# toposware/schnorr-sig

Measured on NVIDIA B200. Metric: schnorr_verifications_per_sec, higher is better.
Workload: dtype u64 (Goldilocks Fp / Fp6 on 32-bit IMAD, exact)

## Files before the change

schnorr-sig_b200/csrc/schnorr_b200.cu:

```cuda
#include <cuda_runtime.h>

#include <cstdio>
#include <cstdlib>
#include <cstring>
#include <string>
#include <vector>

#include "../../include/cheetah_params.h"
#include "../../include/schnorr_b200.h"
#include "verify.cuh"
#include "keyset.cuh"
#include "dist.cuh"
#include "debug_ops.cuh"
#include "derive.cuh"

using namespace sb;

static constexpr size_t GTAB_U64 = (size_t)GTAB_WINDOWS * GTAB_ENTRIES * 12;
static constexpr size_t REG_BATCH_MIN_PER_KEY = 64;

enum scratch_slot { SL_A = 0, SL_B, SL_C, SL_D, SL_E, SL_F, SL_G, SL_H, SL_I, SL_J, SL_K, SL_L, SL_M, SL_N, SL_O, SL_COUNT };

struct schnorr_b200_ctx {
    int device = 0;
    cudaStream_t stream = nullptr;
    cudaStream_t own_stream = nullptr;
    uint64_t* gtab = nullptr;
    void* scratch[SL_COUNT] = {};
    size_t scratch_cap[SL_COUNT] = {};
    uint64_t launches = 0;
    int sm_count = 148;
    cudaEvent_t ev_k0 = nullptr, ev_k1 = nullptr;
    size_t verify_wave = 148 * 256;
    cudaStream_t copy_stream = nullptr;
    cudaStream_t aux_stream = nullptr;
    cudaEvent_t ev_aux = nullptr;
    bool exact_only = false;
    int msm_c_override = 0;
    uint32_t msm_t_override = 0;
    int last_msm_c = 0, last_msm_K = 0;
    uint32_t last_msm_T = 0;
    uint64_t last_batch_points = 0;
    size_t reg_batch_min_per_key = REG_BATCH_MIN_PER_KEY;
    size_t dist_max = 10240;
    size_t one_max = 512;
    size_t batch_dist_max = (size_t)1 << 18;
    size_t batch_small_max = 256;
    int exact_counters_used = 0;
    static constexpr int MAX_CHUNKS = 16;
    cudaEvent_t ev_chunk[MAX_CHUNKS] = {};
    std::string err;
    std::vector<schnorr_b200_ctx*> shards;
};

#define CUDA_TRY(ctx, expr)                                                                      \
    do {                                                                                         \
        cudaError_t e_ = (expr);                                                                 \
        if (e_ != cudaSuccess) {                                                                 \
            (ctx)->err = std::string(#expr) + ": " + cudaGetErrorString(e_);                     \
            return SCHNORR_B200_ECUDA;                                                           \
        }                                                                                        \
    } while (0)

static int ensure_scratch(schnorr_b200_ctx* ctx, int slot, size_t bytes, void** out) {
    if (bytes == 0) bytes = 16;
    if (ctx->scratch_cap[slot] < bytes) {
        if (ctx->scratch[slot]) {
            CUDA_TRY(ctx, cudaStreamSynchronize(ctx->stream));
            CUDA_TRY(ctx, cudaFree(ctx->scratch[slot]));
            ctx->scratch[slot] = nullptr;
            ctx->scratch_cap[slot] = 0;
        }
        size_t cap = bytes + bytes / 8;
        CUDA_TRY(ctx, cudaMalloc(&ctx->scratch[slot], cap));
        ctx->scratch_cap[slot] = cap;
    }
    *out = ctx->scratch[slot];
    return 0;
}

static constexpr uint8_t FL_PK_INF = 1;
static constexpr uint8_t FL_X_BAD = 2;
static constexpr uint8_t FL_MALFORMED = 4;
static constexpr int SOA_PLANES = 11;

struct soa_batch {
    ulonglong2* planes;
    uint8_t* flags;
    uint8_t* sig_flag;
    size_t n;
};

__device__ __forceinline__ ulonglong2 load_plane(const ulonglong2* p) {
    return __ldcs(p);
}
__device__ __forceinline__ fp6 load_fp6_planes(const ulonglong2* planes, int first_plane, size_t n, size_t i) {
    ulonglong2 a = load_plane(&planes[(size_t)(first_plane + 0) * n + i]);
    ulonglong2 b = load_plane(&planes[(size_t)(first_plane + 1) * n + i]);
    ulonglong2 c = load_plane(&planes[(size_t)(first_plane + 2) * n + i]);
    return fp6{{a.x, a.y, b.x, b.y, c.x, c.y}};
}
__device__ __forceinline__ scalar load_scalar_planes(const ulonglong2* planes, int first_plane, size_t n, size_t i) {
    ulonglong2 a = load_plane(&planes[(size_t)(first_plane + 0) * n + i]);
    ulonglong2 b = load_plane(&planes[(size_t)(first_plane + 1) * n + i]);
    return sc_from_u64x4(a.x, a.y, b.x, b.y);
}
__device__ __forceinline__ uint64_t load_u64_le(const uint8_t* p) {
    uint64_t v = 0;
#pragma unroll
    for (int k = 0; k < 8; k++) v |= (uint64_t)p[k] << (8 * k);
    return v;
}

struct hash_vote {
    bool sync, any;
};
__device__ __forceinline__ hash_vote block_hash_vote(int np, uint64_t& off, uint64_t& len) {
    __shared__ int s_np_min, s_np_max, s_first;
    __shared__ uint64_t s_off, s_len;
    if (threadIdx.x == 0) {
        s_np_min = 1 << 30;
        s_np_max = -1;
        s_first = 1 << 30;
    }
    __syncthreads();
    if (np >= 0) {
        atomicMin(&s_np_min, np);
        atomicMax(&s_np_max, np);
        atomicMin(&s_first, (int)threadIdx.x);
    }
    __syncthreads();
    if ((int)threadIdx.x == s_first) {
        s_off = off;
        s_len = len;
    }
    __syncthreads();
    hash_vote v;
    v.any = s_np_max >= 0;
    v.sync = v.any && s_np_min >= s_np_max;
    if (np < 0 && v.any) {
        off = s_off;
        len = s_len;
    }
    return v;
}

static constexpr int INGEST_THREADS = 128;
__global__ void __launch_bounds__(INGEST_THREADS) k_ingest(size_t n, const uint8_t* __restrict__ sigs81,
                                                           const uint8_t* __restrict__ pk96,
                                                           const uint8_t* __restrict__ pk_inf, soa_batch out) {
    __shared__ __align__(16) uint8_t s_sig[INGEST_THREADS * 81];
    size_t base = (size_t)blockIdx.x * INGEST_THREADS;
    size_t cnt = n - base < (size_t)INGEST_THREADS ? n - base : (size_t)INGEST_THREADS;
    size_t bytes = cnt * 81;
    const uint8_t* src = sigs81 + base * 81;
    if ((reinterpret_cast<uintptr_t>(src) & 15) == 0) {
        size_t nv = bytes / 16;
        for (size_t k = threadIdx.x; k < nv; k += INGEST_THREADS)
            reinterpret_cast<uint4*>(s_sig)[k] = reinterpret_cast<const uint4*>(src)[k];
        for (size_t k = nv * 16 + threadIdx.x; k < bytes; k += INGEST_THREADS) s_sig[k] = src[k];
    } else {
        for (size_t k = threadIdx.x; k < bytes; k += INGEST_THREADS) s_sig[k] = src[k];
    }
    __syncthreads();
    size_t i = base + threadIdx.x;
    if (i >= n) return;
    const uint8_t* rec = s_sig + threadIdx.x * 81;
    uint64_t x[6], e[4];
#pragma unroll
    for (int k = 0; k < 6; k++) x[k] = load_u64_le(rec + 8 * k);
#pragma unroll
    for (int k = 0; k < 4; k++) e[k] = load_u64_le(rec + 49 + 8 * k);
    const uint64_t* pk = reinterpret_cast<const uint64_t*>(pk96 + i * 96);
    uint64_t p[12];
#pragma unroll
    for (int k = 0; k < 12; k++) p[k] = pk[k];
    uint8_t fl = 0;
    bool inf = pk_inf != nullptr && pk_inf[i] != 0;
    if (inf) fl |= FL_PK_INF;
    bool x_ok = true, pk_ok = true;
#pragma unroll
    for (int k = 0; k < 6; k++) x_ok &= x[k] < FP_P;
#pragma unroll
    for (int k = 0; k < 12; k++) pk_ok &= p[k] < FP_P;
    if (!x_ok) fl |= FL_X_BAD;
    if ((!pk_ok && !inf) || sc_geq_q(sc_from_u64x4(e[0], e[1], e[2], e[3]))) fl |= FL_MALFORMED;
    size_t N = out.n;
    ulonglong2* pl = out.planes;
    pl[0 * N + i] = make_ulonglong2(x[0], x[1]);
    pl[1 * N + i] = make_ulonglong2(x[2], x[3]);
    pl[2 * N + i] = make_ulonglong2(x[4], x[5]);
    pl[3 * N + i] = make_ulonglong2(e[0], e[1]);
    pl[4 * N + i] = make_ulonglong2(e[2], e[3]);
#pragma unroll
    for (int k = 0; k < 6; k++) pl[(size_t)(5 + k) * N + i] = make_ulonglong2(p[2 * k], p[2 * k + 1]);
    out.flags[i] = fl;
    out.sig_flag[i] = rec[48];
}

#ifndef VERIFY_THREADS_N
#define VERIFY_THREADS_N 128
#endif
static constexpr int VERIFY_THREADS = VERIFY_THREADS_N;
#ifndef VERIFY_MIN_BLOCKS
#define VERIFY_MIN_BLOCKS 2
#endif
__global__ void __launch_bounds__(VERIFY_THREADS, VERIFY_MIN_BLOCKS) k_verify(soa_batch in, const uint8_t* __restrict__ msgs,
                                                           const uint64_t* __restrict__ msg_off,
                                                           const uint64_t* __restrict__ gtab,
                                                           uint8_t* __restrict__ verdicts,
                                                           const uint32_t* __restrict__ work_list,
                                                           const uint32_t* __restrict__ work_count) {
    struct d_slot {
        jac_pt p;
        uint64_t pad;
    };
    __shared__ d_slot s_d[VERIFY_THREADS];
    size_t i = (size_t)blockIdx.x * blockDim.x + threadIdx.x;
    if (work_list) {
        if (i >= *work_count) return;
        i = work_list[i];
    }
    if (i >= in.n) return;
    uint8_t fl = in.flags[i];
    if (fl & FL_MALFORMED) {
        verdicts[i] = VERDICT_MALFORMED;
        return;
    }
    fp6 sx = load_fp6_planes(in.planes, 0, in.n, i);
    scalar e = load_scalar_planes(in.planes, 3, in.n, i);
    fp6 px = load_fp6_planes(in.planes, 5, in.n, i);
    fp6 py = load_fp6_planes(in.planes, 8, in.n, i);
    bool pk_inf = fl & FL_PK_INF;
    bool x_ok = !(fl & FL_X_BAD);
    uint64_t off = msg_off[i];
    scalar h = sc_zero();
    if (x_ok) h = challenge_scalar(sx, px, py, pk_inf, msgs + off, msg_off[i + 1] - off);
    verdicts[i] = verify_points(sx, x_ok, e, px, py, pk_inf, h, gtab, &s_d[threadIdx.x].p);
}

#ifndef VERIFY_FAST_MIN_BLOCKS
#define VERIFY_FAST_MIN_BLOCKS 2
#endif
static constexpr size_t VERIFY_FAST_SMEM = (size_t)(1 + FAST_BH_SHARED) * VERIFY_THREADS * sizeof(jf_pt);
__global__ void __launch_bounds__(VERIFY_THREADS, VERIFY_FAST_MIN_BLOCKS) k_verify_fast(soa_batch in, const uint8_t* __restrict__ msgs,
                                                           const uint64_t* __restrict__ msg_off,
                                                           const uint64_t* __restrict__ gtab,
                                                           uint8_t* __restrict__ verdicts,
                                                           uint32_t* __restrict__ work_list,
                                                           uint32_t* __restrict__ work_count) {
    extern __shared__ __align__(16) unsigned char s_fast[];
    jf_pt* s_d = reinterpret_cast<jf_pt*>(s_fast);
    jf_pt* s_bh = s_d + VERIFY_THREADS;
    size_t i = (size_t)blockIdx.x * blockDim.x + threadIdx.x;
    bool live = i < in.n;
    uint8_t fl = live ? in.flags[i] : FL_MALFORMED;
    bool work = live && !(fl & (FL_MALFORMED | FL_PK_INF));
    uint64_t off = work ? msg_off[i] : 0, len = work ? msg_off[i + 1] - off : 0;
    hash_vote hv = block_hash_vote(work ? hash_message_permutations(len) : -1, off, len);
    fp6 sx = fp6_zero(), px, py;
    scalar e = sc_zero();
    if (work) {
        sx = load_fp6_planes(in.planes, 0, in.n, i);
        e = load_scalar_planes(in.planes, 3, in.n, i);
        px = load_fp6_planes(in.planes, 5, in.n, i);
        py = load_fp6_planes(in.planes, 8, in.n, i);
    } else {
        const uint64_t* g = gtab + (size_t)1 * GTAB_ENTRY_U64;
#pragma unroll
        for (int k = 0; k < 6; k++) {
            px.c[k] = g[k];
            py.c[k] = g[6 + k];
        }
    }
    bool x_ok = !(fl & FL_X_BAD);
    scalar h = sc_zero();
    if (hv.any) {
        h = challenge_scalar(sx, px, py, false, msgs + off, len, hv.sync);
        if (!x_ok || !work) h = sc_zero();
    }
    uint8_t v = verify_points_fast(sx, x_ok, e, px, py, false, h, gtab, s_d + threadIdx.x, s_bh + threadIdx.x, VERIFY_THREADS);
    if (!live) return;
    if (fl & FL_MALFORMED) v = VERDICT_MALFORMED;
    else if (fl & FL_PK_INF) v = VERDICT_NEEDS_EXACT;
    verdicts[i] = v;
    if (v == VERDICT_NEEDS_EXACT) work_list[atomicAdd(work_count, 1u)] = (uint32_t)i;
}

static constexpr int DIST_THREADS = 128;
static constexpr int DIST_SIGS_PER_BLOCK = (DIST_THREADS / 32) * 5;
__global__ void __launch_bounds__(DIST_THREADS) k_verify_dist(soa_batch in, const uint8_t* __restrict__ msgs,
                                                              const uint64_t* __restrict__ msg_off,
                                                              const uint64_t* __restrict__ gtab,
                                                              uint8_t* __restrict__ verdicts,
                                                              uint32_t* __restrict__ work_list,
                                                              uint32_t* __restrict__ work_count) {
    __shared__ uint32_t s_mds2[24];
    if (threadIdx.x < 24) s_mds2[threadIdx.x] = c_mds_row[threadIdx.x % 12];
    __syncthreads();
    int lane = threadIdx.x & 31, warp = threadIdx.x >> 5;
    int g = lane / 6, k = lane % 6;
    if (g >= 5) return;
    size_t i = ((size_t)blockIdx.x * (DIST_THREADS / 32) + warp) * 5 + g;
    if (i >= in.n) return;
    int gbase = 6 * g;
    unsigned mask = 0x3fu << gbase;
    uint8_t fl = in.flags[i];
    if (fl & FL_MALFORMED) {
        if (k == 0) verdicts[i] = VERDICT_MALFORMED;
        return;
    }
    uint8_t v;
    if (fl & FL_PK_INF) {
        v = VERDICT_NEEDS_EXACT;
    } else {
        bool x_ok = !(fl & FL_X_BAD);
        const uint64_t* pl = reinterpret_cast<const uint64_t*>(in.planes);
        size_t n = in.n;
        fp_t sx = pl[((size_t)(0 + (k >> 1)) * n + i) * 2 + (k & 1)];
        fp_t px = pl[((size_t)(5 + (k >> 1)) * n + i) * 2 + (k & 1)];
        fp_t py = pl[((size_t)(8 + (k >> 1)) * n + i) * 2 + (k & 1)];
        scalar e = load_scalar_planes(in.planes, 3, n, i);
        uint64_t off = msg_off[i];
        scalar h = sc_zero();
        if (x_ok) h = dchallenge_scalar(mask, sx, px, py, msgs + off, msg_off[i + 1] - off, k, gbase, s_mds2);
        dpt r;
        int fr = dverify_core(mask, px, py, h, e, gtab, &r, k, gbase);
        bool eq = dall(mask, gbase, r.X == fp_mul(sx, fp_sqr_nc(r.w)));
        v = fr == FAST_EXCEPTIONAL ? VERDICT_NEEDS_EXACT
            : (fr == FAST_NOT_TORSION_FREE ? VERDICT_INVALID_PUBLIC_KEY
               : (!x_ok ? VERDICT_MALFORMED : (eq ? VERDICT_OK : VERDICT_INVALID_SIGNATURE)));
    }
    if (k == 0) {
        verdicts[i] = v;
        if (v == VERDICT_NEEDS_EXACT) work_list[atomicAdd(work_count, 1u)] = (uint32_t)i;
    }
}


static constexpr int HASH_THREADS = 128;
__global__ void __launch_bounds__(HASH_THREADS) k_hash(size_t n, const uint8_t* __restrict__ rx48,
                                                       const uint8_t* __restrict__ pk96,
                                                       const uint8_t* __restrict__ msgs,
                                                       const uint64_t* __restrict__ msg_off,
                                                       uint8_t* __restrict__ digests) {
    size_t i = (size_t)blockIdx.x * blockDim.x + threadIdx.x;
    bool live = i < n;
    uint64_t off = live ? msg_off[i] : 0, len = live ? msg_off[i + 1] - off : 0;
    hash_vote hv = block_hash_vote(live ? hash_message_permutations(len) : -1, off, len);
    size_t src = live ? i : (size_t)blockIdx.x * blockDim.x;
    const uint64_t* r = reinterpret_cast<const uint64_t*>(rx48 + src * 48);
    const uint64_t* p = reinterpret_cast<const uint64_t*>(pk96 + src * 96);
    fp6 rx, px;
#pragma unroll
    for (int k = 0; k < 6; k++) {
        rx.c[k] = r[k];
        px.c[k] = p[k];
    }
    fp_t py0 = p[6];
    fp_t d[4];
    hash_message(rx, px, py0, msgs + off, len, d, hv.sync);
    if (!live) return;
    ulonglong2* o = reinterpret_cast<ulonglong2*>(digests + i * 32);
    o[0] = make_ulonglong2(d[0], d[1]);
    o[1] = make_ulonglong2(d[2], d[3]);
}

__global__ void __launch_bounds__(DIST_THREADS) k_hash_dist(size_t n, const uint8_t* __restrict__ rx48,
                                                            const uint8_t* __restrict__ pk96,
                                                            const uint8_t* __restrict__ msgs,
                                                            const uint64_t* __restrict__ msg_off,
                                                            uint8_t* __restrict__ digests) {
    __shared__ uint32_t s_mds2[24];
    if (threadIdx.x < 24) s_mds2[threadIdx.x] = c_mds_row[threadIdx.x % 12];
    __syncthreads();
    int lane = threadIdx.x & 31, warp = threadIdx.x >> 5;
    int g = lane / 6, k = lane % 6;
    if (g >= 5) return;
    size_t i = ((size_t)blockIdx.x * (DIST_THREADS / 32) + warp) * 5 + g;
    if (i >= n) return;
    int gbase = 6 * g;
    unsigned mask = 0x3fu << gbase;
    const uint64_t* r = reinterpret_cast<const uint64_t*>(rx48 + i * 48);
    const uint64_t* p = reinterpret_cast<const uint64_t*>(pk96 + i * 96);
    uint64_t off = msg_off[i];
    fp_t d[4];
    dhash_message(mask, r[k], p[k], p[6 + k], msgs + off, msg_off[i + 1] - off, k, gbase, s_mds2, d);
    if (k < 4) reinterpret_cast<uint64_t*>(digests + i * 32)[k] = d[k];
}

static constexpr int SIGN_THREADS = 128;
__device__ __forceinline__ void store_point96(uint8_t* dst, const fp6& x, const fp6& y) {
    uint64_t* o = reinterpret_cast<uint64_t*>(dst);
#pragma unroll
    for (int k = 0; k < 6; k++) {
        o[k] = x.c[k];
        o[6 + k] = y.c[k];
    }
}
__global__ void __launch_bounds__(SIGN_THREADS) k_keygen(size_t n, const uint8_t* __restrict__ sk32,
                                                         const uint64_t* __restrict__ gtab, uint8_t* __restrict__ pk96,
                                                         uint8_t* __restrict__ pk_inf) {
    size_t i = (size_t)blockIdx.x * blockDim.x + threadIdx.x;
    if (i >= n) return;
    scalar k = sc_from_u256(sc_load_le(sk32 + 32 * i));
    jac_pt P = fixed_base_mul(k, gtab);
    fp6 x, y;
    bool inf;
    jac_to_affine(P, x, y, inf);
    store_point96(pk96 + 96 * i, x, y);
    if (pk_inf) pk_inf[i] = inf ? 1 : 0;
}
__global__ void __launch_bounds__(SIGN_THREADS) k_sign(size_t n, const uint8_t* __restrict__ sk32,
                                                       const uint8_t* __restrict__ pk96,
                                                       const uint8_t* __restrict__ pk_inf,
                                                       const uint8_t* __restrict__ msgs,
                                                       const uint64_t* __restrict__ msg_off,
                                                       const uint8_t* __restrict__ nonce32,
                                                       const uint64_t* __restrict__ gtab, uint8_t* __restrict__ sigs81) {
    size_t i = (size_t)blockIdx.x * blockDim.x + threadIdx.x;
    if (i >= n) return;
    scalar sk = sc_from_u256(sc_load_le(sk32 + 32 * i));
    scalar r = sc_from_u256(sc_load_le(nonce32 + 32 * i));
    const uint64_t* p = reinterpret_cast<const uint64_t*>(pk96 + i * 96);
    fp6 px, py;
#pragma unroll
    for (int k = 0; k < 6; k++) {
        px.c[k] = p[k];
        py.c[k] = p[6 + k];
    }
    bool inf = pk_inf != nullptr && pk_inf[i] != 0;
    jac_pt R = fixed_base_mul(r, gtab);
    fp6 x, y;
    bool r_inf;
    jac_to_affine(R, x, y, r_inf);
    uint64_t off = msg_off[i];
    scalar h = challenge_scalar(x, px, py, inf, msgs + off, msg_off[i + 1] - off);
    scalar e = sc_sub(r, sc_mul(sk, h));
    uint8_t* o = sigs81 + 81 * i;
#pragma unroll
    for (int k = 0; k < 6; k++)
#pragma unroll
        for (int b = 0; b < 8; b++) o[8 * k + b] = (uint8_t)(x.c[k] >> (8 * b));
    o[48] = compress_flags(y, r_inf);
#pragma unroll
    for (int k = 0; k < 8; k++)
#pragma unroll
        for (int b = 0; b < 4; b++) o[49 + 4 * k + b] = (uint8_t)(e.l[k] >> (8 * b));
}

__global__ void __launch_bounds__(128) k_decompress(size_t n, const uint8_t* __restrict__ in49, uint8_t* __restrict__ pk96,
                                                    uint8_t* __restrict__ pk_inf, uint8_t* __restrict__ ok) {
    size_t i = (size_t)blockIdx.x * blockDim.x + threadIdx.x;
    if (i >= n) return;
    const uint8_t* rec = in49 + 49 * i;
    fp6 x;
#pragma unroll
    for (int k = 0; k < 6; k++) x.c[k] = load_u64_le(rec + 8 * k);
    fp6 ox, oy;
    bool inf;
    bool good = decompress_point(x, rec[48], ox, oy, inf);
    store_point96(pk96 + 96 * i, ox, oy);
    pk_inf[i] = inf ? 1 : 0;
    ok[i] = good ? 1 : 0;
}
__global__ void __launch_bounds__(128) k_compress(size_t n, const uint8_t* __restrict__ pk96,
                                                  const uint8_t* __restrict__ pk_inf, uint8_t* __restrict__ out49) {
    size_t i = (size_t)blockIdx.x * blockDim.x + threadIdx.x;
    if (i >= n) return;
    const uint64_t* p = reinterpret_cast<const uint64_t*>(pk96 + i * 96);
    bool inf = pk_inf != nullptr && pk_inf[i] != 0;
    fp6 y;
#pragma unroll
    for (int k = 0; k < 6; k++) y.c[k] = p[6 + k];
    uint8_t* o = out49 + 49 * i;
#pragma unroll
    for (int k = 0; k < 6; k++) {
        uint64_t v = inf ? 0 : p[k];
#pragma unroll
        for (int b = 0; b < 8; b++) o[8 * k + b] = (uint8_t)(v >> (8 * b));
    }
    o[48] = compress_flags(y, inf);
}

__global__ void __launch_bounds__(128) k_split_keyed(size_t n, const uint8_t* __restrict__ keyed130, uint8_t* __restrict__ pk96,
                                                     uint8_t* __restrict__ pk_inf, uint8_t* __restrict__ ok,
                                                     uint8_t* __restrict__ sigs81) {
    size_t i = (size_t)blockIdx.x * blockDim.x + threadIdx.x;
    if (i >= n) return;
    const uint8_t* rec = keyed130 + 130 * i;
    fp6 x;
#pragma unroll
    for (int k = 0; k < 6; k++) x.c[k] = load_u64_le(rec + 8 * k);
    fp6 ox, oy;
    bool inf;
    bool good = decompress_point(x, rec[48], ox, oy, inf);
    store_point96(pk96 + 96 * i, ox, oy);
    pk_inf[i] = inf ? 1 : 0;
    ok[i] = good ? 1 : 0;
    for (int k = 0; k < 81; k++) sigs81[81 * i + k] = rec[49 + k];
}
__global__ void k_mask_verdicts(size_t n, const uint8_t* __restrict__ ok, uint8_t* __restrict__ verdicts) {
    size_t i = (size_t)blockIdx.x * blockDim.x + threadIdx.x;
    if (i < n && !ok[i]) verdicts[i] = VERDICT_MALFORMED;
}

__global__ void __launch_bounds__(128) k_derive_master(size_t n, const uint8_t* __restrict__ seeds32, uint8_t* __restrict__ xsk64,
                                                       uint8_t* __restrict__ ok) {
    size_t i = (size_t)blockIdx.x * blockDim.x + threadIdx.x;
    if (i >= n) return;
    ok[i] = derive_master(seeds32 + 32 * i, xsk64 + 64 * i) ? 1 : 0;
}
__global__ void __launch_bounds__(128) k_derive_private(size_t n, const uint8_t* __restrict__ parent_xsk64,
                                                        const uint8_t* __restrict__ parent49, const uint32_t* __restrict__ indices,
                                                        uint8_t* __restrict__ children64, uint8_t* __restrict__ ok) {
    size_t i = (size_t)blockIdx.x * blockDim.x + threadIdx.x;
    if (i >= n) return;
    ok[i] = derive_private_child(parent_xsk64, parent49, indices[i], children64 + 64 * i) ? 1 : 0;
}
__global__ void k_parent_public(const uint8_t* __restrict__ parent_xsk64, const uint64_t* __restrict__ gtab, uint8_t* __restrict__ out49) {
    if (blockIdx.x != 0 || threadIdx.x != 0) return;
    scalar k = sc_from_u256(sc_load_le(parent_xsk64));
    jac_pt P = fixed_base_mul(k, gtab);
    fp6 x, y;
    bool inf;
    jac_to_affine(P, x, y, inf);
    for (int c = 0; c < 6; c++)
        for (int b = 0; b < 8; b++) out49[8 * c + b] = (uint8_t)((inf ? 0 : x.c[c]) >> (8 * b));
    out49[48] = compress_flags(y, inf);
}
__global__ void __launch_bounds__(SIGN_THREADS) k_derive_public(size_t n, const uint8_t* __restrict__ parent_xpk81,
                                                                const uint8_t* __restrict__ parent96,
                                                                const uint8_t* __restrict__ parent_inf,
                                                                const uint32_t* __restrict__ indices,
                                                                const uint64_t* __restrict__ gtab, uint8_t* __restrict__ children81,
                                                                uint8_t* __restrict__ ok) {
    size_t i = (size_t)blockIdx.x * blockDim.x + threadIdx.x;
    if (i >= n) return;
    uint32_t index = indices[i];
    uint8_t* o = children81 + 81 * i;
    scalar t = derive_public_tweak(parent_xpk81, parent_xpk81 + 49, index, o + 49);
    const uint64_t* p = reinterpret_cast<const uint64_t*>(parent96);
    fp6 px, py;
#pragma unroll
    for (int k = 0; k < 6; k++) {
        px.c[k] = p[k];
        py.c[k] = p[6 + k];
    }
    jac_pt acc = fixed_base_mul(t, gtab);
    bool tweak_inf = jac_is_identity(acc);
    acc = jac_madd(acc, px, py, parent_inf[0] != 0);
    fp6 x, y;
    bool inf;
    jac_to_affine(acc, x, y, inf);
#pragma unroll
    for (int k = 0; k < 6; k++)
#pragma unroll
        for (int b = 0; b < 8; b++) o[8 * k + b] = (uint8_t)((inf ? 0 : x.c[k]) >> (8 * b));
    o[48] = compress_flags(y, inf);
    ok[i] = (!tweak_inf && (index >> 31) == 0) ? 1 : 0;
}

__global__ void __launch_bounds__(128) k_tab_bases(size_t n_pts, const uint64_t* __restrict__ pts12, const uint8_t* __restrict__ skip,
                                                   int w, int windows, jac_pt* __restrict__ bases) {
    size_t p = (size_t)blockIdx.x * blockDim.x + threadIdx.x;
    if (p >= n_pts || (skip && skip[p])) return;
    tab_bases(pts12 + 12 * p, w, windows, bases + p * windows);
}
__global__ void __launch_bounds__(128) k_tab_fill(size_t n_pts, const uint8_t* __restrict__ skip, int w, int windows,
                                                  const jac_pt* __restrict__ bases, uint64_t* __restrict__ tab) {
    size_t t = (size_t)blockIdx.x * blockDim.x + threadIdx.x;
    size_t entries = ((size_t)1 << (w - 1)) + 1, per_pt = (size_t)windows * entries;
    if (t >= n_pts * per_pt) return;
    size_t p = t / per_pt;
    if (skip && skip[p]) return;
    tab_entry(bases[t / entries], w, (int)(t % entries), tab + t * 12);
}

__global__ void __launch_bounds__(128) k_keyset_register(size_t n_keys, const uint64_t* __restrict__ pk12,
                                                         const uint8_t* __restrict__ pk_inf, uint8_t* __restrict__ status,
                                                         uint8_t* __restrict__ skip) {
    size_t k = (size_t)blockIdx.x * blockDim.x + threadIdx.x;
    if (k >= n_keys) return;
    bool inf = pk_inf[k] != 0;
    jac_pt d;
    uint8_t st = keyset_key_status(pk12 + 12 * k, inf, &d);
    status[k] = st;
    skip[k] = st != KEY_OK || inf;
}
__global__ void __launch_bounds__(128) k_keyset_gather(size_t n, const uint32_t* __restrict__ key_idx, size_t n_keys,
                                                       const uint64_t* __restrict__ ks_pk12, const uint8_t* __restrict__ ks_inf,
                                                       uint64_t* __restrict__ pk12, uint8_t* __restrict__ pk_inf) {
    size_t i = (size_t)blockIdx.x * blockDim.x + threadIdx.x;
    if (i >= n) return;
    uint32_t k = key_idx[i];
    bool in = k < n_keys;
#pragma unroll
    for (int c = 0; c < 12; c++) pk12[12 * i + c] = in ? ks_pk12[12 * (size_t)k + c] : ~0ULL;
    pk_inf[i] = in ? ks_inf[k] : 0;
}
__global__ void __launch_bounds__(128) k_keyset_encode(size_t n_keys, const uint64_t* __restrict__ pk12,
                                                       const uint8_t* __restrict__ pk_inf, keyset_entry* __restrict__ entries,
                                                       uint8_t* __restrict__ findable) {
    size_t k = (size_t)blockIdx.x * blockDim.x + threadIdx.x;
    if (k >= n_keys) return;
    keyset_entry e;
    uint8_t flag;
    findable[k] = keyset_encode(pk12 + 12 * k, pk_inf[k] != 0, e.x, flag) ? 1 : 0;
    e.flag = flag;
    e.index = (uint32_t)k;
    e.pad = 0;
    entries[k] = e;
}
__global__ void __launch_bounds__(128) k_keyset_lookup(size_t n, const uint8_t* __restrict__ keys49,
                                                       const keyset_entry* __restrict__ lut, uint32_t n_lut,
                                                       uint32_t* __restrict__ key_idx) {
    size_t i = (size_t)blockIdx.x * blockDim.x + threadIdx.x;
    if (i >= n) return;
    const uint8_t* rec = keys49 + 49 * i;
    uint64_t x[6];
#pragma unroll
    for (int k = 0; k < 6; k++) x[k] = load_u64_le(rec + 8 * k);
    key_idx[i] = keyset_lookup(lut, n_lut, x, rec[48]);
}
__global__ void __launch_bounds__(128) k_keyed_split_lookup(size_t n, const uint8_t* __restrict__ keyed130,
                                                            const keyset_entry* __restrict__ lut, uint32_t n_lut,
                                                            const uint64_t* __restrict__ ks_pk12,
                                                            const uint8_t* __restrict__ ks_inf, uint8_t* __restrict__ pk96,
                                                            uint8_t* __restrict__ pk_inf, uint8_t* __restrict__ ok,
                                                            uint8_t* __restrict__ sigs81, uint32_t* __restrict__ key_idx,
                                                            uint32_t* __restrict__ miss_count) {
    size_t i = (size_t)blockIdx.x * blockDim.x + threadIdx.x;
    bool miss = false;
    if (i < n) {
        const uint8_t* rec = keyed130 + 130 * i;
        fp6 x;
#pragma unroll
        for (int k = 0; k < 6; k++) x.c[k] = load_u64_le(rec + 8 * k);
        uint32_t k = keyset_lookup(lut, n_lut, x.c, rec[48]);
        miss = k == KEYSET_MISS;
        if (!miss) {
            uint64_t* o = reinterpret_cast<uint64_t*>(pk96 + 96 * i);
#pragma unroll
            for (int c = 0; c < 12; c++) o[c] = ks_pk12[12 * (size_t)k + c];
            pk_inf[i] = ks_inf[k];
            ok[i] = 1;
        } else {
            fp6 ox, oy;
            bool inf;
            bool good = decompress_point(x, rec[48], ox, oy, inf);
            store_point96(pk96 + 96 * i, ox, oy);
            pk_inf[i] = inf ? 1 : 0;
            ok[i] = good ? 1 : 0;
        }
        key_idx[i] = k;
        for (int c = 0; c < 81; c++) sigs81[81 * i + c] = rec[49 + c];
    }
    unsigned m = __ballot_sync(0xffffffffu, miss);
    if ((threadIdx.x & 31) == 0 && m) atomicAdd(miss_count, (unsigned)__popc(m));
}

template <bool LOOKUP>
__global__ void __launch_bounds__(VERIFY_THREADS) k_verify_reg(soa_batch in, const uint32_t* __restrict__ key_idx,
                                                               const uint8_t* __restrict__ key_status,
                                                               const uint64_t* __restrict__ ktab,
                                                               const uint8_t* __restrict__ msgs,
                                                               const uint64_t* __restrict__ msg_off,
                                                               const uint64_t* __restrict__ gtab,
                                                               uint8_t* __restrict__ verdicts,
                                                               uint32_t* __restrict__ work_list,
                                                               uint32_t* __restrict__ work_count) {
    size_t i = (size_t)blockIdx.x * blockDim.x + threadIdx.x;
    bool live = i < in.n;
    uint8_t fl = live ? in.flags[i] : FL_MALFORMED;
    bool keyed = !(fl & (FL_MALFORMED | FL_PK_INF));
    uint32_t k = keyed ? key_idx[i] : 0;
    bool miss = LOOKUP && k == KEYSET_MISS;
    if (miss) {
        keyed = false;
        k = 0;
    }
    uint8_t st = keyed ? key_status[k] : KEY_OK;
    bool work = keyed && st == KEY_OK;
    uint64_t off = work ? msg_off[i] : 0, len = work ? msg_off[i + 1] - off : 0;
    hash_vote hv = block_hash_vote(work ? hash_message_permutations(len) : -1, off, len);
    fp6 sx = fp6_zero(), px, py;
    scalar e = sc_zero();
    if (work) {
        sx = load_fp6_planes(in.planes, 0, in.n, i);
        e = load_scalar_planes(in.planes, 3, in.n, i);
        px = load_fp6_planes(in.planes, 5, in.n, i);
        py = load_fp6_planes(in.planes, 8, in.n, i);
    } else {
        const uint64_t* g = gtab + (size_t)1 * GTAB_ENTRY_U64;
#pragma unroll
        for (int c = 0; c < 6; c++) {
            px.c[c] = g[c];
            py.c[c] = g[6 + c];
        }
    }
    bool x_ok = !(fl & FL_X_BAD);
    scalar h = sc_zero();
    if (hv.any) {
        h = challenge_scalar(sx, px, py, false, msgs + off, len, hv.sync);
        if (!x_ok || !work) h = sc_zero();
    }
    jf_pt r;
    int fr = verify_core_reg(h, e, ktab + (size_t)k * KT_KEY_U64, gtab, &r);
    if (!live) return;
    uint8_t v;
    if (fl & FL_MALFORMED) v = VERDICT_MALFORMED;
    else if (fl & FL_PK_INF) v = VERDICT_NEEDS_EXACT;
    else if (miss) v = VERDICT_NEEDS_EXACT;
    else v = reg_verdict(st, x_ok, fr, r, sx);
    verdicts[i] = v;
    if (v == VERDICT_NEEDS_EXACT) work_list[atomicAdd(work_count, 1u)] = (uint32_t)i;
}

__global__ void __launch_bounds__(128) k_debug_field(size_t n, const uint64_t* __restrict__ a6, const uint64_t* __restrict__ b6,
                                                     uint64_t* __restrict__ out48) {
    size_t i = (size_t)blockIdx.x * blockDim.x + threadIdx.x;
    if (i >= n) return;
    fp6 a, b;
#pragma unroll
    for (int k = 0; k < 6; k++) {
        a.c[k] = a6[i * 6 + k];
        b.c[k] = b6[i * 6 + k];
    }
    fp6 m = fp6_mul(a, b), q = fp6_sqr(a), ad = fp6_add(a, b), su = fp6_sub(a, b), iv = fp6_inv(a);
    uint64_t* o = out48 + i * 48;
#pragma unroll
    for (int k = 0; k < 6; k++) {
        o[k] = m.c[k];
        o[6 + k] = q.c[k];
        o[12 + k] = ad.c[k];
        o[18 + k] = su.c[k];
        o[24 + k] = fp_mul(a.c[k], b.c[k]);
        o[30 + k] = fp_sqr(a.c[k]);
        o[36 + k] = iv.c[k];
        o[42 + k] = rescue_inv_sbox(a.c[k]);
    }
}

__global__ void __launch_bounds__(128) k_debug_lazy(size_t n, const uint64_t* __restrict__ a6, const uint64_t* __restrict__ b6,
                                                    uint64_t* __restrict__ out48) {
    size_t i = (size_t)blockIdx.x * blockDim.x + threadIdx.x;
    if (i >= n) return;
    fp6 a, b, r[8];
#pragma unroll
    for (int k = 0; k < 6; k++) {
        a.c[k] = a6[i * 6 + k];
        b.c[k] = b6[i * 6 + k];
    }
    debug_lazy_ops(a, b, r);
    for (int j = 0; j < 8; j++)
        for (int k = 0; k < 6; k++) out48[i * 48 + 6 * j + k] = r[j].c[k];
}

__global__ void __launch_bounds__(256) k_imad_peak(int iters, uint64_t* sink) {
    uint32_t a = threadIdx.x * 2654435761u + 12345u, b = blockIdx.x * 40503u + 977u;
    uint64_t acc[8];
#pragma unroll
    for (int k = 0; k < 8; k++) acc[k] = k;
    for (int it = 0; it < iters; it++) {
#pragma unroll
        for (int k = 0; k < 8; k++) {
            asm volatile("mad.wide.u32 %0, %1, %2, %0;" : "+l"(acc[k]) : "r"(a + k), "r"(b));
        }
        b += 3;
    }
    uint64_t s = 0;
#pragma unroll
    for (int k = 0; k < 8; k++) s ^= acc[k];
    if (s == 0x123456789abcdefULL) sink[0] = s;
}

static inline unsigned grid_for(size_t n, int threads) { return (unsigned)((n + threads - 1) / threads); }

static int build_tables(schnorr_b200_ctx* ctx, size_t n_pts, const uint64_t* pts12, const uint8_t* skip, int w, int windows,
                        jac_pt* bases, uint64_t* tab) {
    size_t threads = n_pts * (size_t)windows * (((size_t)1 << (w - 1)) + 1);
    k_tab_bases<<<grid_for(n_pts, 128), 128, 0, ctx->stream>>>(n_pts, pts12, skip, w, windows, bases);
    k_tab_fill<<<grid_for(threads, 128), 128, 0, ctx->stream>>>(n_pts, skip, w, windows, bases, tab);
    ctx->launches += 2;
    CUDA_TRY(ctx, cudaGetLastError());
    return 0;
}

static int alloc_soa(schnorr_b200_ctx* ctx, size_t n, soa_batch* b) {
    void *p, *f, *sf;
    if (int rc = ensure_scratch(ctx, SL_A, sizeof(ulonglong2) * SOA_PLANES * n, &p)) return rc;
    if (int rc = ensure_scratch(ctx, SL_B, n, &f)) return rc;
    if (int rc = ensure_scratch(ctx, SL_C, n, &sf)) return rc;
    b->planes = (ulonglong2*)p;
    b->flags = (uint8_t*)f;
    b->sig_flag = (uint8_t*)sf;
    b->n = n;
    return 0;
}

static bool msg_off_valid(size_t n, const uint64_t* msg_off) {
    if (msg_off[0] != 0) return false;
    for (size_t i = 0; i < n; i++)
        if (msg_off[i + 1] < msg_off[i]) return false;
    return true;
}
#define CHECK_MSG_OFF(ctx, n, msg_off)                                                            \
    do {                                                                                          \
        if (!msg_off_valid((n), (msg_off))) {                                                     \
            (ctx)->err = "message offsets must start at 0 and be non-decreasing";                 \
            return SCHNORR_B200_EARG;                                                             \
        }                                                                                         \
    } while (0)

static int stage_in(schnorr_b200_ctx* ctx, int slot, const void* host, size_t bytes, void** dev) {
    if (int rc = ensure_scratch(ctx, slot, bytes, dev)) return rc;
    if (host && bytes) CUDA_TRY(ctx, cudaMemcpyAsync(*dev, host, bytes, cudaMemcpyHostToDevice, ctx->stream));
    return 0;
}

#define MULTI_DISPATCH(ctx, call)                                  \
    do {                                                           \
        if ((ctx) && !(ctx)->shards.empty()) return call;          \
    } while (0)
#define NOT_ON_MULTI(ctx)                                                                                          \
    do {                                                                                                           \
        if ((ctx) && !(ctx)->shards.empty()) {                                                                     \
            (ctx)->err = "device-pointer entry points need a single-device context (buffers live on one device)"; \
            return SCHNORR_B200_EARG;                                                                              \
        }                                                                                                          \
    } while (0)

static int verify_many_host(schnorr_b200_ctx* ctx, size_t n, const uint8_t* sigs81, const uint8_t* pk96, const uint8_t* pk_inf,
                            const uint8_t* msgs, const uint64_t* msg_off, uint8_t* verdicts, bool validate_offsets);
#include "batch.cuh"
#include "multi.cuh"
#include "one.cuh"


static int launch_verify(schnorr_b200_ctx* ctx, const soa_batch& soa, const uint8_t* msgs, const uint64_t* msg_off,
                         uint8_t* verdicts, size_t list_base, int counter, size_t list_total, cudaStream_t st) {
    unsigned grid = grid_for(soa.n, VERIFY_THREADS);
    if (counter == 0) ctx->exact_counters_used = 0;
    if (ctx->exact_only) {
        k_verify<<<grid, VERIFY_THREADS, 0, st>>>(soa, msgs, msg_off, ctx->gtab, verdicts, nullptr, nullptr);
        ctx->launches += 1;
        return 0;
    }
    void* wl;
    if (int rc = ensure_scratch(ctx, SL_M, 4 * (list_total + schnorr_b200_ctx::MAX_CHUNKS), &wl)) return rc;
    uint32_t* counters = (uint32_t*)wl;
    uint32_t* list = counters + schnorr_b200_ctx::MAX_CHUNKS + list_base;
    CUDA_TRY(ctx, cudaMemsetAsync(counters + counter, 0, 4, st));
    if (counter + 1 > ctx->exact_counters_used) ctx->exact_counters_used = counter + 1;
    if (soa.n <= ctx->one_max)
        if (soa.n <= (size_t)2 * ctx->sm_count)
            k_verify_one<2><<<(unsigned)soa.n, ONE_THREADS, 0, st>>>(soa, msgs, msg_off, ctx->gtab, verdicts, list, counters + counter);
        else
            k_verify_one<4><<<(unsigned)soa.n, ONE_THREADS, 0, st>>>(soa, msgs, msg_off, ctx->gtab, verdicts, list, counters + counter);
    else if (soa.n <= ctx->dist_max)
        k_verify_dist<<<grid_for(soa.n, DIST_SIGS_PER_BLOCK), DIST_THREADS, 0, st>>>(soa, msgs, msg_off, ctx->gtab, verdicts, list,
                                                                                   counters + counter);
    else
        k_verify_fast<<<grid, VERIFY_THREADS, VERIFY_FAST_SMEM, st>>>(soa, msgs, msg_off, ctx->gtab, verdicts, list, counters + counter);
    k_verify<<<grid, VERIFY_THREADS, 0, st>>>(soa, msgs, msg_off, ctx->gtab, verdicts, list, counters + counter);
    ctx->launches += 2;
    return 0;
}

extern "C" {

int schnorr_b200_params_pinned(void) { return CHEETAH_PARAMS_PINNED; }
const char* schnorr_b200_params_provenance(void) { return CHEETAH_PARAMS_PROVENANCE; }

int schnorr_b200_create(int device, schnorr_b200_ctx** out) {
    if (!out) return SCHNORR_B200_EARG;
    *out = nullptr;
#if !CHEETAH_PARAMS_PINNED
    {
        static bool warned = false;
        if (!warned) {
            warned = true;
            fprintf(stderr, "schnorr_b200: curve / hash parameters are NOT pinned to the upstream cheetah / hash crates (%s). "
                            "Keys and signatures interoperate with the real schnorr-sig crate only after "
                            "rust/dump_params has been run and include/cheetah_params.h regenerated.\n",
                    CHEETAH_PARAMS_PROVENANCE);
        }
    }
#endif
    int count = 0;
    if (cudaGetDeviceCount(&count) != cudaSuccess || count <= 0 || device < 0 || device >= count) {
        (void)cudaGetLastError();
        return SCHNORR_B200_ENODEV;
    }
    schnorr_b200_ctx* ctx = new schnorr_b200_ctx();
    ctx->device = device;
    auto fail = [&](int rc) {
        fprintf(stderr, "schnorr_b200_create: %s\n", ctx->err.c_str());
        schnorr_b200_destroy(ctx);
        return rc;
    };
#define CREATE_TRY(expr)                                                          \
    do {                                                                          \
        cudaError_t e_ = (expr);                                                  \
        if (e_ != cudaSuccess) {                                                  \
            ctx->err = std::string(#expr) + ": " + cudaGetErrorString(e_);        \
            return fail(SCHNORR_B200_ECUDA);                                      \
        }                                                                         \
    } while (0)
    CREATE_TRY(cudaSetDevice(device));
    cudaDeviceProp prop;
    CREATE_TRY(cudaGetDeviceProperties(&prop, device));
    ctx->sm_count = prop.multiProcessorCount;
    CREATE_TRY(cudaStreamCreateWithFlags(&ctx->own_stream, cudaStreamNonBlocking));
    ctx->stream = ctx->own_stream;
    {
        int per_sm = 0;
        CREATE_TRY(cudaFuncSetAttribute(k_verify_fast, cudaFuncAttributeMaxDynamicSharedMemorySize, (int)VERIFY_FAST_SMEM));
        CREATE_TRY(cudaFuncSetAttribute(k_verify_fast, cudaFuncAttributePreferredSharedMemoryCarveout, cudaSharedmemCarveoutMaxShared));
        CREATE_TRY(cudaOccupancyMaxActiveBlocksPerMultiprocessor(&per_sm, k_verify_fast, VERIFY_THREADS, VERIFY_FAST_SMEM));
        if (per_sm < 1) per_sm = 1;
        ctx->verify_wave = (size_t)ctx->sm_count * per_sm * VERIFY_THREADS;
    }
    CREATE_TRY(cudaStreamCreateWithFlags(&ctx->copy_stream, cudaStreamNonBlocking));
    CREATE_TRY(cudaStreamCreateWithFlags(&ctx->aux_stream, cudaStreamNonBlocking));
    CREATE_TRY(cudaEventCreateWithFlags(&ctx->ev_aux, cudaEventDisableTiming));
    for (int c = 0; c < schnorr_b200_ctx::MAX_CHUNKS; c++) CREATE_TRY(cudaEventCreateWithFlags(&ctx->ev_chunk[c], cudaEventDisableTiming));
    CREATE_TRY(cudaEventCreate(&ctx->ev_k0));
    CREATE_TRY(cudaEventCreate(&ctx->ev_k1));
    CREATE_TRY(cudaMemcpyToSymbol(c_ark, RESCUE_ARK, sizeof(uint64_t) * 2 * RESCUE_ROUNDS * 12));
    CREATE_TRY(cudaMemcpyToSymbol(c_q_wnaf5, CHEETAH_Q_WNAF5, sizeof(CHEETAH_Q_WNAF5)));
    CREATE_TRY(cudaMemcpyToSymbol(c_q_wnaf4, CHEETAH_Q_WNAF4, 256));
    CREATE_TRY(cudaMalloc(&ctx->gtab, GTAB_U64 * sizeof(uint64_t)));
    jac_pt* bases = nullptr;
    CREATE_TRY(cudaMalloc(&bases, sizeof(jac_pt) * GTAB_WINDOWS + 96));
    uint64_t* g12 = reinterpret_cast<uint64_t*>(bases + GTAB_WINDOWS);
    CREATE_TRY(cudaMemcpyAsync(g12, CHEETAH_GX, 48, cudaMemcpyHostToDevice, ctx->stream));
    CREATE_TRY(cudaMemcpyAsync(g12 + 6, CHEETAH_GY, 48, cudaMemcpyHostToDevice, ctx->stream));
    if (build_tables(ctx, 1, g12, nullptr, GTAB_W, GTAB_WINDOWS, bases, ctx->gtab)) {
        cudaFree(bases);
        return fail(SCHNORR_B200_ECUDA);
    }
    CREATE_TRY(cudaStreamSynchronize(ctx->stream));
    cudaFree(bases);
#undef CREATE_TRY
    *out = ctx;
    return SCHNORR_B200_OK;
}

int schnorr_b200_create_multi(const int* devices, int n_devices, schnorr_b200_ctx** out) {
    if (!out) return SCHNORR_B200_EARG;
    *out = nullptr;
    if (!devices || n_devices <= 0 || n_devices > 64) return SCHNORR_B200_EARG;
    if (n_devices == 1) return schnorr_b200_create(devices[0], out);
    schnorr_b200_ctx* ctx = new schnorr_b200_ctx();
    ctx->device = devices[0];
    for (int k = 0; k < n_devices; k++) {
        schnorr_b200_ctx* sh = nullptr;
        int rc = schnorr_b200_create(devices[k], &sh);
        if (rc != SCHNORR_B200_OK) {
            schnorr_b200_destroy(ctx);
            return rc;
        }
        ctx->shards.push_back(sh);
    }
    ctx->sm_count = ctx->shards[0]->sm_count;
    ctx->verify_wave = ctx->shards[0]->verify_wave;
    *out = ctx;
    return SCHNORR_B200_OK;
}
int schnorr_b200_device_count(const schnorr_b200_ctx* ctx) { return !ctx ? 0 : (ctx->shards.empty() ? 1 : (int)ctx->shards.size()); }

void schnorr_b200_destroy(schnorr_b200_ctx* ctx) {
    if (!ctx) return;
    if (!ctx->shards.empty()) {
        for (schnorr_b200_ctx* sh : ctx->shards) schnorr_b200_destroy(sh);
        delete ctx;
        return;
    }
    cudaSetDevice(ctx->device);
    if (ctx->own_stream) cudaStreamSynchronize(ctx->own_stream);
    for (int s = 0; s < SL_COUNT; s++)
        if (ctx->scratch[s]) cudaFree(ctx->scratch[s]);
    if (ctx->gtab) cudaFree(ctx->gtab);
    for (int c = 0; c < schnorr_b200_ctx::MAX_CHUNKS; c++)
        if (ctx->ev_chunk[c]) cudaEventDestroy(ctx->ev_chunk[c]);
    if (ctx->copy_stream) cudaStreamDestroy(ctx->copy_stream);
    if (ctx->aux_stream) cudaStreamDestroy(ctx->aux_stream);
    if (ctx->ev_aux) cudaEventDestroy(ctx->ev_aux);
    if (ctx->ev_k0) cudaEventDestroy(ctx->ev_k0);
    if (ctx->ev_k1) cudaEventDestroy(ctx->ev_k1);
    if (ctx->own_stream) cudaStreamDestroy(ctx->own_stream);
    delete ctx;
}

const char* schnorr_b200_last_error(const schnorr_b200_ctx* ctx) { return ctx ? ctx->err.c_str() : "null context"; }

int schnorr_b200_set_stream(schnorr_b200_ctx* ctx, void* stream) {
    if (!ctx) return SCHNORR_B200_EARG;
    NOT_ON_MULTI(ctx);
    ctx->stream = stream ? (cudaStream_t)stream : ctx->own_stream;
    return SCHNORR_B200_OK;
}
int schnorr_b200_synchronize(schnorr_b200_ctx* ctx) {
    if (!ctx) return SCHNORR_B200_EARG;
    for (schnorr_b200_ctx* sh : ctx->shards)
        if (int rc = schnorr_b200_synchronize(sh)) return rc;
    if (!ctx->shards.empty()) return SCHNORR_B200_OK;
    CUDA_TRY(ctx, cudaStreamSynchronize(ctx->stream));
    return SCHNORR_B200_OK;
}
uint64_t schnorr_b200_launch_count(const schnorr_b200_ctx* ctx) {
    if (!ctx) return 0;
    uint64_t total = ctx->launches;
    for (const schnorr_b200_ctx* sh : ctx->shards) total += sh->launches;
    return total;
}
int schnorr_b200_last_kernel_ms(schnorr_b200_ctx* ctx, float* ms) {
    if (!ctx || !ms) return SCHNORR_B200_EARG;
    if (!ctx->shards.empty()) {
        *ms = 0;
        for (schnorr_b200_ctx* sh : ctx->shards) {
            float m = 0;
            if (int rc = schnorr_b200_last_kernel_ms(sh, &m)) return rc;
            if (m > *ms) *ms = m;
        }
        return SCHNORR_B200_OK;
    }
    CUDA_TRY(ctx, cudaEventSynchronize(ctx->ev_k1));
    CUDA_TRY(ctx, cudaEventElapsedTime(ms, ctx->ev_k0, ctx->ev_k1));
    return SCHNORR_B200_OK;
}

int schnorr_b200_set_exact_only(schnorr_b200_ctx* ctx, int exact_only) {
    if (!ctx) return SCHNORR_B200_EARG;
    for (schnorr_b200_ctx* sh : ctx->shards) sh->exact_only = exact_only != 0;
    ctx->exact_only = exact_only != 0;
    return SCHNORR_B200_OK;
}
int schnorr_b200_set_dist_threshold(schnorr_b200_ctx* ctx, size_t max_signatures) {
    if (!ctx) return SCHNORR_B200_EARG;
    for (schnorr_b200_ctx* sh : ctx->shards) sh->dist_max = max_signatures;
    ctx->dist_max = max_signatures;
    return SCHNORR_B200_OK;
}
int schnorr_b200_set_one_threshold(schnorr_b200_ctx* ctx, size_t max_signatures) {
    if (!ctx) return SCHNORR_B200_EARG;
    for (schnorr_b200_ctx* sh : ctx->shards) sh->one_max = max_signatures;
    ctx->one_max = max_signatures;
    return SCHNORR_B200_OK;
}
int schnorr_b200_set_batch_small_threshold(schnorr_b200_ctx* ctx, size_t max_signatures) {
    if (!ctx) return SCHNORR_B200_EARG;
    for (schnorr_b200_ctx* sh : ctx->shards) sh->batch_small_max = max_signatures;
    ctx->batch_small_max = max_signatures;
    return SCHNORR_B200_OK;
}
int schnorr_b200_set_batch_dist_threshold(schnorr_b200_ctx* ctx, size_t max_signatures) {
    if (!ctx) return SCHNORR_B200_EARG;
    ctx->batch_dist_max = max_signatures;
    for (schnorr_b200_ctx* sh : ctx->shards) sh->batch_dist_max = max_signatures;
    return SCHNORR_B200_OK;
}
int schnorr_b200_set_msm_geometry(schnorr_b200_ctx* ctx, int window_bits, unsigned segment_len) {
    if (!ctx || (window_bits != 0 && (window_bits < 4 || window_bits > 16)) || (segment_len != 0 && segment_len < 8))
        return SCHNORR_B200_EARG;
    ctx->msm_c_override = window_bits;
    ctx->msm_t_override = segment_len;
    for (schnorr_b200_ctx* sh : ctx->shards) {
        sh->msm_c_override = window_bits;
        sh->msm_t_override = segment_len;
    }
    return SCHNORR_B200_OK;
}
int schnorr_b200_last_batch_plan(const schnorr_b200_ctx* ctx, int* window_bits, int* windows, unsigned* segment_len) {
    if (!ctx) return SCHNORR_B200_EARG;
    const schnorr_b200_ctx* c = ctx->shards.empty() ? ctx : ctx->shards[0];
    if (window_bits) *window_bits = c->last_msm_c;
    if (windows) *windows = c->last_msm_K;
    if (segment_len) *segment_len = c->last_msm_T;
    return SCHNORR_B200_OK;
}
int schnorr_b200_last_batch_points(const schnorr_b200_ctx* ctx, uint64_t* points) {
    if (!ctx || !points) return SCHNORR_B200_EARG;
    *points = ctx->last_batch_points;
    return SCHNORR_B200_OK;
}
int schnorr_b200_set_registered_batch_threshold(schnorr_b200_ctx* ctx, size_t min_signatures_per_key) {
    if (!ctx) return SCHNORR_B200_EARG;
    ctx->reg_batch_min_per_key = min_signatures_per_key;
    for (schnorr_b200_ctx* sh : ctx->shards) sh->reg_batch_min_per_key = min_signatures_per_key;
    return SCHNORR_B200_OK;
}
int schnorr_b200_last_exact_count(schnorr_b200_ctx* ctx, uint64_t* count) {
    if (!ctx || !count) return SCHNORR_B200_EARG;
    *count = 0;
    if (!ctx->shards.empty()) {
        for (schnorr_b200_ctx* sh : ctx->shards) {
            uint64_t c = 0;
            if (int rc = schnorr_b200_last_exact_count(sh, &c)) return rc;
            *count += c;
        }
        return SCHNORR_B200_OK;
    }
    if (ctx->exact_counters_used == 0 || !ctx->scratch[SL_M]) return SCHNORR_B200_OK;
    uint32_t c[schnorr_b200_ctx::MAX_CHUNKS] = {};
    CUDA_TRY(ctx, cudaSetDevice(ctx->device));
    CUDA_TRY(ctx, cudaStreamSynchronize(ctx->stream));
    CUDA_TRY(ctx, cudaMemcpy(c, ctx->scratch[SL_M], 4 * ctx->exact_counters_used, cudaMemcpyDeviceToHost));
    for (int i = 0; i < ctx->exact_counters_used; i++) *count += c[i];
    return SCHNORR_B200_OK;
}

int schnorr_b200_hash_messages_dev(schnorr_b200_ctx* ctx, size_t n, const uint8_t* rx48, const uint8_t* pk96,
                                   const uint8_t* msgs, const uint64_t* msg_off, uint8_t* digests) {
    NOT_ON_MULTI(ctx);
    if (!ctx || (n && (!rx48 || !pk96 || !msg_off || !digests))) return SCHNORR_B200_EARG;
    if (n == 0) return SCHNORR_B200_OK;
    CUDA_TRY(ctx, cudaSetDevice(ctx->device));
    cudaEventRecord(ctx->ev_k0, ctx->stream);
    if (n <= ctx->dist_max)
        k_hash_dist<<<grid_for(n, DIST_SIGS_PER_BLOCK), DIST_THREADS, 0, ctx->stream>>>(n, rx48, pk96, msgs, msg_off, digests);
    else
        k_hash<<<grid_for(n, HASH_THREADS), HASH_THREADS, 0, ctx->stream>>>(n, rx48, pk96, msgs, msg_off, digests);
    cudaEventRecord(ctx->ev_k1, ctx->stream);
    ctx->launches += 1;
    CUDA_TRY(ctx, cudaGetLastError());
    return SCHNORR_B200_OK;
}

int schnorr_b200_hash_messages(schnorr_b200_ctx* ctx, size_t n, const uint8_t* rx48, const uint8_t* pk96,
                               const uint8_t* msgs, const uint64_t* msg_off, uint8_t* digests) {
    MULTI_DISPATCH(ctx, multi_hash_messages(ctx, n, rx48, pk96, msgs, msg_off, digests));
    if (!ctx || (n && (!rx48 || !pk96 || !msg_off || !digests))) return SCHNORR_B200_EARG;
    if (n == 0) return SCHNORR_B200_OK;
    CUDA_TRY(ctx, cudaSetDevice(ctx->device));
    CHECK_MSG_OFF(ctx, n, msg_off);
    size_t mb = msg_off[n];
    if (mb && !msgs) return SCHNORR_B200_EARG;
    void *d_rx, *d_pk, *d_m, *d_off, *d_out;
    if (int rc = stage_in(ctx, SL_D, rx48, n * 48, &d_rx)) return rc;
    if (int rc = stage_in(ctx, SL_E, pk96, n * 96, &d_pk)) return rc;
    if (int rc = stage_in(ctx, SL_F, msgs, mb, &d_m)) return rc;
    if (int rc = stage_in(ctx, SL_G, msg_off, (n + 1) * 8, &d_off)) return rc;
    if (int rc = ensure_scratch(ctx, SL_H, n * 32, &d_out)) return rc;
    if (int rc = schnorr_b200_hash_messages_dev(ctx, n, (uint8_t*)d_rx, (uint8_t*)d_pk, (uint8_t*)d_m, (uint64_t*)d_off,
                                                (uint8_t*)d_out))
        return rc;
    CUDA_TRY(ctx, cudaMemcpyAsync(digests, d_out, n * 32, cudaMemcpyDeviceToHost, ctx->stream));
    CUDA_TRY(ctx, cudaStreamSynchronize(ctx->stream));
    return SCHNORR_B200_OK;
}

int schnorr_b200_verify_many_dev(schnorr_b200_ctx* ctx, size_t n, const uint8_t* sigs81, const uint8_t* pk96,
                                 const uint8_t* pk_inf, const uint8_t* msgs, const uint64_t* msg_off,
                                 uint8_t* verdicts) {
    NOT_ON_MULTI(ctx);
    if (!ctx || (n && (!sigs81 || !pk96 || !msg_off || !verdicts))) return SCHNORR_B200_EARG;
    if (n == 0) return SCHNORR_B200_OK;
    CUDA_TRY(ctx, cudaSetDevice(ctx->device));
    soa_batch soa;
    if (int rc = alloc_soa(ctx, n, &soa)) return rc;
    k_ingest<<<grid_for(n, INGEST_THREADS), INGEST_THREADS, 0, ctx->stream>>>(n, sigs81, pk96, pk_inf, soa);
    cudaEventRecord(ctx->ev_k0, ctx->stream);
    if (int rc = launch_verify(ctx, soa, msgs, msg_off, verdicts, 0, 0, n, ctx->stream)) return rc;
    cudaEventRecord(ctx->ev_k1, ctx->stream);
    ctx->launches += 1;
// ... 868 lines not shown
```

Baseline: 14.01 million.

## Split challenge hashing out of fast verify into a separate kernel

Adds a k_challenge kernel that computes the Poseidon challenge scalar per signature and writes it into two new SoA planes. k_verify_fast then loads h from memory instead of hashing inline, which shrinks its register footprint and removes hash-related divergence from the point-verification kernel. The cost is an extra launch plus extra global traffic for the h planes. It also relies on the SoA allocation being sized for 13 planes, and only py.c[0] is passed to the hash, which assumes the challenge uses nothing else from py.

```diff
diff --git a/schnorr-sig_b200/csrc/schnorr_b200.cu b/schnorr-sig_b200/csrc/schnorr_b200.cu
--- a/schnorr-sig_b200/csrc/schnorr_b200.cu
+++ b/schnorr-sig_b200/csrc/schnorr_b200.cu
@@ -82,7 +82,8 @@
 static constexpr uint8_t FL_PK_INF = 1;
 static constexpr uint8_t FL_X_BAD = 2;
 static constexpr uint8_t FL_MALFORMED = 4;
-static constexpr int SOA_PLANES = 11;
+static constexpr int SOA_PLANES = 13;
+static constexpr int SOA_H_PLANE = 11;
 
 struct soa_batch {
     ulonglong2* planes;
@@ -239,12 +240,36 @@
     verdicts[i] = verify_points(sx, x_ok, e, px, py, pk_inf, h, gtab, &s_d[threadIdx.x].p);
 }
 
+static constexpr int CHALLENGE_THREADS = 128;
+__global__ void __launch_bounds__(CHALLENGE_THREADS, 4) k_challenge(soa_batch in, const uint8_t* __restrict__ msgs,
+                                                                    const uint64_t* __restrict__ msg_off) {
+    size_t i = (size_t)blockIdx.x * blockDim.x + threadIdx.x;
+    bool live = i < in.n;
+    uint8_t fl = live ? in.flags[i] : FL_MALFORMED;
+    bool work = live && !(fl & (FL_MALFORMED | FL_PK_INF));
+    uint64_t off = work ? msg_off[i] : 0, len = work ? msg_off[i + 1] - off : 0;
+    hash_vote hv = block_hash_vote(work ? hash_message_permutations(len) : -1, off, len);
+    fp6 sx = fp6_zero(), px = fp6_zero(), py = fp6_zero();
+    if (work) {
+        sx = load_fp6_planes(in.planes, 0, in.n, i);
+        px = load_fp6_planes(in.planes, 5, in.n, i);
+        py.c[0] = in.planes[(size_t)8 * in.n + i].x;
+    }
+    scalar h = sc_zero();
+    if (hv.any) {
+        h = challenge_scalar(sx, px, py, false, msgs + off, len, hv.sync);
+        if (!work || (fl & FL_X_BAD)) h = sc_zero();
+    }
+    if (!live) return;
+    in.planes[(size_t)(SOA_H_PLANE + 0) * in.n + i] = make_ulonglong2(sc_u64(h, 0), sc_u64(h, 1));
+    in.planes[(size_t)(SOA_H_PLANE + 1) * in.n + i] = make_ulonglong2(sc_u64(h, 2), sc_u64(h, 3));
+}
+
 #ifndef VERIFY_FAST_MIN_BLOCKS
 #define VERIFY_FAST_MIN_BLOCKS 2
 #endif
 static constexpr size_t VERIFY_FAST_SMEM = (size_t)(1 + FAST_BH_SHARED) * VERIFY_THREADS * sizeof(jf_pt);
-__global__ void __launch_bounds__(VERIFY_THREADS, VERIFY_FAST_MIN_BLOCKS) k_verify_fast(soa_batch in, const uint8_t* __restrict__ msgs,
-                                                           const uint64_t* __restrict__ msg_off,
+__global__ void __launch_bounds__(VERIFY_THREADS, VERIFY_FAST_MIN_BLOCKS) k_verify_fast(soa_batch in,
                                                            const uint64_t* __restrict__ gtab,
                                                            uint8_t* __restrict__ verdicts,
                                                            uint32_t* __restrict__ work_list,
@@ -256,15 +281,14 @@
     bool live = i < in.n;
     uint8_t fl = live ? in.flags[i] : FL_MALFORMED;
     bool work = live && !(fl & (FL_MALFORMED | FL_PK_INF));
-    uint64_t off = work ? msg_off[i] : 0, len = work ? msg_off[i + 1] - off : 0;
-    hash_vote hv = block_hash_vote(work ? hash_message_permutations(len) : -1, off, len);
     fp6 sx = fp6_zero(), px, py;
-    scalar e = sc_zero();
+    scalar e = sc_zero(), h = sc_zero();
     if (work) {
         sx = load_fp6_planes(in.planes, 0, in.n, i);
         e = load_scalar_planes(in.planes, 3, in.n, i);
         px = load_fp6_planes(in.planes, 5, in.n, i);
         py = load_fp6_planes(in.planes, 8, in.n, i);
+        h = load_scalar_planes(in.planes, SOA_H_PLANE, in.n, i);
     } else {
         const uint64_t* g = gtab + (size_t)1 * GTAB_ENTRY_U64;
 #pragma unroll
@@ -274,11 +298,6 @@
         }
     }
     bool x_ok = !(fl & FL_X_BAD);
-    scalar h = sc_zero();
-    if (hv.any) {
-        h = challenge_scalar(sx, px, py, false, msgs + off, len, hv.sync);
-        if (!x_ok || !work) h = sc_zero();
-    }
     uint8_t v = verify_points_fast(sx, x_ok, e, px, py, false, h, gtab, s_d + threadIdx.x, s_bh + threadIdx.x, VERIFY_THREADS);
     if (!live) return;
     if (fl & FL_MALFORMED) v = VERDICT_MALFORMED;
@@ -861,8 +880,11 @@
     else if (soa.n <= ctx->dist_max)
         k_verify_dist<<<grid_for(soa.n, DIST_SIGS_PER_BLOCK), DIST_THREADS, 0, st>>>(soa, msgs, msg_off, ctx->gtab, verdicts, list,
                                                                                    counters + counter);
-    else
-        k_verify_fast<<<grid, VERIFY_THREADS, VERIFY_FAST_SMEM, st>>>(soa, msgs, msg_off, ctx->gtab, verdicts, list, counters + counter);
+    else {
+        k_challenge<<<grid_for(soa.n, CHALLENGE_THREADS), CHALLENGE_THREADS, 0, st>>>(soa, msgs, msg_off);
+        k_verify_fast<<<grid, VERIFY_THREADS, VERIFY_FAST_SMEM, st>>>(soa, ctx->gtab, verdicts, list, counters + counter);
+        ctx->launches += 1;
+    }
     k_verify<<<grid, VERIFY_THREADS, 0, st>>>(soa, msgs, msg_off, ctx->gtab, verdicts, list, counters + counter);
     ctx->launches += 2;
     return 0;
```

Measured after the change: 14.31 million, median of 6. 1.02x the previous value.
